# bjo5029/causal-vae

Measured on AMD Instinct MI355X. Metric: training samples/sec on 128^3 vessel volumes (3D CausalVAE train step), higher is better.
Workload: dtype bf16; 1 GPU; 3D vessel CausalVAE train step, 128^3 bf16 volumes (z-scored N(0,1)), batch 4/GPU, Adam lr 0.0001, ELBO = MSE-sum + 2000*MSE-sum(m) + KLD; global_batch=4, per_gpu_batch=4, parallelism=dp1, params=15346957

## Files before the change

causal_vae_amd/csrc/bottleneck.hip:

```cpp
#include "common.h"

#define BN_MAXM 16

namespace {

CVAE_TUNABLE(BN_NT, 0);
CVAE_TUNABLE(BN_FWD_UNROLL, 2);
CVAE_TUNABLE(BN_BWD_UNROLL, 8);
CVAE_TUNABLE(BN_FWD_SLICE, 4096);
CVAE_TUNABLE(BN_BWD_ROWS, 16);

struct TailDims { int M, N1, N2, Z, T, HM, DM, KS, P, NZ; };
struct TailParams {
    const float *b1, *W2, *b2, *Wmu, *bmu, *Wlv, *blv, *Wm0, *bm0, *gamma, *beta, *Wm3, *bm3, *Wm5, *bm5;
};
struct TailGrads {
    float *db1, *dW2, *db2, *dWmu, *dbmu, *dWlv, *dblv, *dWm0, *dbm0, *dgamma, *dbeta, *dWm3, *dbm3, *dWm5, *dbm5;
};
struct TailSaved { float *h1, *h2, *mu, *logvar, *xhat, *invstd, *a1n, *a2, *m_hat, *zm; };
struct MechFwdArgs { const float* t_onehot; float *running_mean, *running_var; long long* num_batches_tracked; float momentum, bn_eps; int bn_training;
                     const float* sync_stats; int sync_ranks; };
struct MechBwdArgs { const float *dzm_part, *g_mhat, *t_onehot; float *sync_dy, *sync_local; };
struct __attribute__((packed, aligned(4))) F4U { float x, y, z, w; };
typedef float v4f_u __attribute__((ext_vector_type(4), aligned(4)));
typedef float v2f_u __attribute__((ext_vector_type(2), aligned(4)));
struct F2U;
template <typename V> __device__ __forceinline__ V ld_stream(const float* p) {
    if constexpr (BN_NT & 1) {
        if constexpr (sizeof(V) == 16) { const v4f_u v = __builtin_nontemporal_load((const v4f_u*)p); V r; __builtin_memcpy(&r, &v, 16); return r; }
        else { const v2f_u v = __builtin_nontemporal_load((const v2f_u*)p); V r; __builtin_memcpy(&r, &v, 8); return r; }
    } else return *(const V*)p;
}
template <typename V> __device__ __forceinline__ void st_stream(float* p, const V& val) {
    if constexpr (BN_NT & 2) {
        if constexpr (sizeof(V) == 16) { v4f_u v; __builtin_memcpy(&v, &val, 16); __builtin_nontemporal_store(v, (v4f_u*)p); }
        else { v2f_u v; __builtin_memcpy(&v, &val, 8); __builtin_nontemporal_store(v, (v2f_u*)p); }
    } else *(V*)p = val;
}

template <int U>
__device__ __forceinline__ void copy_g2l(float* __restrict__ dst, const float* __restrict__ src, int n) {
    for (int base = threadIdx.x; base < n; base += 256 * U) {
        float v[U];
#pragma unroll
        for (int u = 0; u < U; ++u) v[u] = src[min(base + 256 * u, n - 1)];
#pragma unroll
        for (int u = 0; u < U; ++u) if (base + 256 * u < n) dst[base + 256 * u] = v[u];
    }
}
__device__ __forceinline__ void copy_rows_g2l(float* __restrict__ ws, const float* __restrict__ wsrc, int n, int K4, int KP) {
    constexpr int U = 8;
    for (int base = threadIdx.x * 4; base < n; base += 1024 * U) {
        float4 v[U];
#pragma unroll
        for (int u = 0; u < U; ++u) v[u] = *(const float4*)(wsrc + min(base + 1024 * u, n - 4));
#pragma unroll
        for (int u = 0; u < U; ++u) {
            const int i = base + 1024 * u;
            if (i < n) {
                const int r = i / K4, k = i - r * K4;
                float* d = ws + r * KP + k;
                d[0] = v[u].x; d[1] = v[u].y; d[2] = v[u].z; d[3] = v[u].w;
            }
        }
    }
}

struct NoiseDraw { float* eps; int n; uint64_t seed, subseq; int* counter; };
template <typename T>
__global__ __launch_bounds__(256) void pool_cat_fwd_kernel(const T* __restrict__ y, const float* __restrict__ m, float* __restrict__ t,
                                                           const long long* __restrict__ t_labels, float* __restrict__ xcat, int D, int H, int W, int C,
                                                           int OD, int OH, int OW, int m_dim, int t_dim, int K1, NoiseDraw nz) {
    const int S = OD * OH * OW, b = blockIdx.y, s = blockIdx.x;
    float* row = xcat + (size_t)b * K1;
    if (s == S) {
        if (nz.counter && b == 0) {
            const uint64_t offset = ((uint64_t)(unsigned)(*nz.counter)) << 24;
            __syncthreads();
            if (threadIdx.x == 0) *nz.counter += 1;
            for (int i = threadIdx.x; i < (nz.n + 3) / 4; i += 256) {
                float v[4];
                philox_normal4(offset + (uint64_t)i, nz.subseq, nz.seed, v);
                for (int j = 0; j < 4; ++j) if (i * 4 + j < nz.n) nz.eps[i * 4 + j] = v[j];
            }
        }
        if (t_labels) {
            const long long lab = t_labels[b];
            for (int i = threadIdx.x; i < t_dim; i += 256) { const float v = (i == lab) ? 1.f : 0.f; t[b * t_dim + i] = v; row[C * S + m_dim + i] = v; }
            for (int i = threadIdx.x; i < m_dim; i += 256) row[C * S + i] = m[b * m_dim + i];
            return;
        }
        for (int i = threadIdx.x; i < m_dim + t_dim; i += 256) row[C * S + i] = i < m_dim ? m[b * m_dim + i] : t[b * t_dim + i - m_dim];
        return;
    }
    const int ow = s % OW, oh = (s / OW) % OH, od = s / (OW * OH);
    const int d0 = pool_lo(od, D, OD), d1 = pool_hi(od, D, OD), h0 = pool_lo(oh, H, OH), h1 = pool_hi(oh, H, OH), w0 = pool_lo(ow, W, OW), w1 = pool_hi(ow, W, OW);
    const float inv = 1.f / (float)((d1 - d0) * (h1 - h0) * (w1 - w0));
    const int nh = h1 - h0, nw = w1 - w0, nvox = (d1 - d0) * nh * nw;
    for (int c = threadIdx.x; c < C; c += 256) {
        float acc = 0.f;
        constexpr int U = 8;
        for (int v0 = 0; v0 < nvox; v0 += U) {
            float v[U];
#pragma unroll
            for (int u = 0; u < U; ++u) {
                const int vi = min(v0 + u, nvox - 1), w = vi % nw, h = (vi / nw) % nh, d = vi / (nw * nh);
                v[u] = to_f32(y[((((size_t)b * D + d0 + d) * H + h0 + h) * W + w0 + w) * C + c]);
            }
#pragma unroll
            for (int u = 0; u < U; ++u) if (v0 + u < nvox) acc += v[u];
        }
        row[c * S + s] = acc * inv;
    }
}

__device__ void mech_fwd(const TailDims& d, const TailParams& p, const TailSaved& sv, const float* __restrict__ t_onehot, float* __restrict__ running_mean,
                         float* __restrict__ running_var, long long* __restrict__ num_batches_tracked, float momentum, float bn_eps, int bn_training, float* lds,
                         const float* __restrict__ sync_stats, int sync_ranks);
__device__ void mech_bwd(const TailDims& d, const TailParams& p, const TailGrads& gr, const TailSaved& sv, const float* __restrict__ dzm_part,
                         const float* __restrict__ g_mhat, const float* __restrict__ t_onehot, float* lds, float* __restrict__ sync_dy, float* __restrict__ sync_local);

template <int MT>
__global__ __launch_bounds__(256) void skinny_fwd_partial_kernel(const float* __restrict__ x, const float* __restrict__ Wt, float* __restrict__ partial,
                                                                 int M, int K, int N, int kslice, int KS, TailDims d, TailParams tp, TailSaved sv, MechFwdArgs ma) {
    extern __shared__ float dyn_lds[];
    if ((int)blockIdx.y == KS) {
        if (blockIdx.x == 0) mech_fwd(d, tp, sv, ma.t_onehot, ma.running_mean, ma.running_var, ma.num_batches_tracked, ma.momentum, ma.bn_eps, ma.bn_training, dyn_lds, ma.sync_stats, ma.sync_ranks);
        return;
    }
    constexpr int R = 4;
    const int n0 = blockIdx.x * R, ks = blockIdx.y;
    const int k0 = ks * kslice, k1 = min(K, k0 + kslice);
    float acc[R][MT];
#pragma unroll
    for (int r = 0; r < R; ++r)
#pragma unroll
        for (int mm = 0; mm < MT; ++mm) acc[r][mm] = 0.f;
    const float* wr[R];
#pragma unroll
    for (int r = 0; r < R; ++r) wr[r] = Wt + (size_t)min(n0 + r, N - 1) * K;
    const int kvec = k0 + ((k1 - k0) & ~3);
#pragma unroll BN_FWD_UNROLL
    for (int k = k0 + 4 * threadIdx.x; k < kvec; k += 1024) {
        F4U xv[MT], wv[R];
#pragma unroll
        for (int mm = 0; mm < MT; ++mm) xv[mm] = mm < M ? *(const F4U*)(x + (size_t)mm * K + k) : F4U{0.f, 0.f, 0.f, 0.f};
#pragma unroll
        for (int r = 0; r < R; ++r) wv[r] = ld_stream<F4U>(wr[r] + k);
#pragma unroll
        for (int r = 0; r < R; ++r)
#pragma unroll
            for (int mm = 0; mm < MT; ++mm) acc[r][mm] += wv[r].x * xv[mm].x + wv[r].y * xv[mm].y + wv[r].z * xv[mm].z + wv[r].w * xv[mm].w;
    }
    for (int k = kvec + threadIdx.x; k < k1; k += 256) {
#pragma unroll
        for (int r = 0; r < R; ++r)
#pragma unroll
            for (int mm = 0; mm < MT; ++mm)
                if (mm < M) acc[r][mm] += wr[r][k] * x[(size_t)mm * K + k];
    }
    __shared__ float red[4][R * MT];
    const int lane = threadIdx.x & 63, wave = threadIdx.x >> 6;
#pragma unroll
    for (int r = 0; r < R; ++r)
#pragma unroll
        for (int mm = 0; mm < MT; ++mm) {
            const float sum = wave_sum(acc[r][mm]);
            if (lane == 0) red[wave][r * MT + mm] = sum;
        }
    __syncthreads();
    if (threadIdx.x < R * MT) {
        const int r = threadIdx.x / MT, mm = threadIdx.x % MT;
        if (mm < M && n0 + r < N)
            partial[((size_t)ks * M + mm) * N + n0 + r] = red[0][threadIdx.x] + red[1][threadIdx.x] + red[2][threadIdx.x] + red[3][threadIdx.x];
    }
}


__device__ void wg_linear_fwd(const float* __restrict__ Wt, const float* __restrict__ bias, const float* xs, float* ys, float* __restrict__ yg,
                              int M, int K, int N, int act) {
    const int lane = threadIdx.x & 63, wave = threadIdx.x >> 6, nw = blockDim.x >> 6;
    for (int n = wave; n < N; n += nw) {
        float acc[BN_MAXM];
#pragma unroll
        for (int m = 0; m < BN_MAXM; ++m) acc[m] = 0.f;
        for (int k = lane; k < K; k += 64) {
            const float w = Wt[(size_t)n * K + k];
#pragma unroll
            for (int m = 0; m < BN_MAXM; ++m)
                if (m < M) acc[m] += w * xs[m * K + k];
        }
#pragma unroll
        for (int m = 0; m < BN_MAXM; ++m) {
            if (m >= M) break;
            const float s = wave_sum(acc[m]);
            if (lane == 0) {
                const float v = apply_act(s + (bias ? bias[n] : 0.f), act);
                ys[m * N + n] = v;
                if (yg) yg[(size_t)m * N + n] = v;
            }
        }
    }
}

__device__ inline float bn_bwd_dx(float k, float nb, float dy, float dbet, float xh, float dgam) { return k * fmaf(-xh, dgam, fmaf(nb, dy, -dbet)); }

__device__ void wg_linear_bwd(const float* __restrict__ Wt, float* __restrict__ dW, float* __restrict__ db, const float* gs, const float* xs, float* dxs,
                              int M, int K, int N) {
    const int T = blockDim.x;
    for (int i = threadIdx.x; i < N * K; i += T) {
        const int n = i / K, k = i - n * K;
        float acc = 0.f;
        for (int m = 0; m < M; ++m) acc += gs[m * N + n] * xs[m * K + k];
        dW[i] = acc;
    }
    if (db)
        for (int n = threadIdx.x; n < N; n += T) {
            float acc = 0.f;
            for (int m = 0; m < M; ++m) acc += gs[m * N + n];
            db[n] = acc;
        }
    if (dxs)
        for (int i = threadIdx.x; i < M * K; i += T) {
            const int m = i / K, k = i - m * K;
            float acc = 0.f;
#pragma unroll 8
            for (int n = 0; n < N; ++n) acc += gs[m * N + n] * Wt[(size_t)n * K + k];
// ... 145 lines not shown
    float* h2s = lds;
    constexpr int HO = 4;
    const int j = blockIdx.x * 4 + wave;
    float wmp[HO], wlp[HO];
#pragma unroll
    for (int u = 0; u < HO; ++u) {
        const size_t o = (size_t)min(j, d.Z - 1) * d.N2 + min(lane + 64 * u, d.N2 - 1);
        wmp[u] = p.Wmu[o]; wlp[u] = p.Wlv[o];
    }
    copy_g2l<4>(h2s, sv.h2, M * d.N2);
    __syncthreads();
    if (j >= d.Z) return;
    float am[BN_MAXM], al[BN_MAXM];
#pragma unroll
    for (int m = 0; m < BN_MAXM; ++m) { am[m] = 0.f; al[m] = 0.f; }
#pragma unroll
    for (int u = 0; u < HO; ++u) {
        const int k = lane + 64 * u;
        if (k < d.N2) {
#pragma unroll
            for (int m = 0; m < BN_MAXM; ++m)
                if (m < M) { am[m] += wmp[u] * h2s[m * d.N2 + k]; al[m] += wlp[u] * h2s[m * d.N2 + k]; }
        }
    }
    for (int k = lane + 64 * HO; k < d.N2; k += 64) {
        const float wm = p.Wmu[(size_t)j * d.N2 + k], wl = p.Wlv[(size_t)j * d.N2 + k];
#pragma unroll
        for (int m = 0; m < BN_MAXM; ++m)
            if (m < M) { am[m] += wm * h2s[m * d.N2 + k]; al[m] += wl * h2s[m * d.N2 + k]; }
    }
#pragma unroll
    for (int m = 0; m < BN_MAXM; ++m) {
        if (m >= M) break;
        const float smu = wave_sum(am[m]), slv = wave_sum(al[m]);
        if (lane == 0) {
            const float mu = smu + p.bmu[j], lv = slv + p.blv[j];
            sv.mu[m * d.Z + j] = mu; sv.logvar[m * d.Z + j] = lv;
            sv.zm[m * K4 + j] = mu + eps[m * d.Z + j] * __expf(0.5f * lv);
        }
    }
}

template <typename T>
__global__ __launch_bounds__(256) void dec_input_fwd_kernel(const float* __restrict__ zm, const float* __restrict__ Wd, const float* __restrict__ bd,
                                                            T* __restrict__ out, int M, int K4, int S, int C) {
    extern __shared__ float lds[];
    const int KP = K4 | 1;
    float* ws = lds;
    float* zs = ws + 64 * KP;
    float* part = zs + M * K4;
    const int tid = threadIdx.x;
    const size_t row0 = (size_t)blockIdx.x * 64;
    const float* wsrc = Wd + row0 * K4;
    if ((K4 & 3) == 0) copy_rows_g2l(ws, wsrc, 64 * K4, K4, KP);
    else {
        for (int i = tid; i < 64 * K4; i += 256) { const int r = i / K4, k = i - r * K4; ws[r * KP + k] = wsrc[i]; }
    }
    copy_g2l<2>(zs, zm, M * K4);
    __syncthreads();
    const int r = tid & 63, q = tid >> 6;
    const int kq = (K4 + 3) / 4, ka = q * kq, kb = min(K4, ka + kq);
    float acc[BN_MAXM];
#pragma unroll
    for (int m = 0; m < BN_MAXM; ++m) acc[m] = 0.f;
    for (int k = ka; k < kb; ++k) {
        const float w = ws[r * KP + k];
#pragma unroll
        for (int m = 0; m < BN_MAXM; ++m)
            if (m < M) acc[m] += w * zs[m * K4 + k];
    }
#pragma unroll
    for (int m = 0; m < BN_MAXM; ++m)
        if (m < M) part[(q * M + m) * 64 + r] = acc[m];
    __syncthreads();
    for (int i = tid; i < M * 64; i += 256) {
        const int m = i >> 6, rr = i & 63;
        const int n = (int)row0 + rr, c = n / S, sc = n - c * S;
        const float v = part[(0 * M + m) * 64 + rr] + part[(1 * M + m) * 64 + rr] + part[(2 * M + m) * 64 + rr] + part[(3 * M + m) * 64 + rr] + bd[n];
        out[((size_t)m * S + sc) * C + c] = from_f32<T>(v);
    }
}

template <typename T>
__global__ __launch_bounds__(256) void dec_input_bwd_kernel(const T* __restrict__ gcl, const float* __restrict__ zm, const float* __restrict__ Wd,
                                                            float* __restrict__ dWd, float* __restrict__ dbd, float* __restrict__ dzm_acc,
                                                            int M, int K4, int S, int C) {
    extern __shared__ float lds[];
    constexpr int R = 64;
    const int KP = K4 | 1;
    float* ws = lds;
    float* zs = ws + R * KP;
    float* gs = zs + M * K4;
    const int tid = threadIdx.x;
    const size_t row0 = (size_t)blockIdx.x * R;
    const float* wsrc = Wd + row0 * K4;
    float* wdst = dWd + row0 * K4;
    const bool v4 = (K4 & 3) == 0;
    {
        constexpr int UG = (BN_MAXM * R) / 256;
        float gv[UG];
#pragma unroll
        for (int u = 0; u < UG; ++u) {
            const int i = min(tid + 256 * u, M * R - 1);
            const int m = i / R, n = (int)row0 + (i - m * R), c = n / S, sc = n - c * S;
            gv[u] = to_f32(gcl[((size_t)m * S + sc) * C + c]);
        }
        if (v4) copy_rows_g2l(ws, wsrc, R * K4, K4, KP);
        else {
            for (int i = tid; i < R * K4; i += 256) { const int r = i / K4, k = i - r * K4; ws[r * KP + k] = wsrc[i]; }
        }
        copy_g2l<2>(zs, zm, M * K4);
#pragma unroll
        for (int u = 0; u < UG; ++u) if (tid + 256 * u < M * R) gs[tid + 256 * u] = gv[u];
    }
    __syncthreads();
    if (v4) {
        for (int i = tid * 4; i < R * K4; i += 1024) {
            const int r = i / K4, k = i - r * K4;
            float4 a = make_float4(0.f, 0.f, 0.f, 0.f);
            for (int m = 0; m < M; ++m) {
                const float gv = gs[m * R + r];
                const float* z = zs + m * K4 + k;
                a.x += gv * z[0]; a.y += gv * z[1]; a.z += gv * z[2]; a.w += gv * z[3];
            }
            *(float4*)(wdst + i) = a;
        }
    } else {
        for (int i = tid; i < R * K4; i += 256) {
            const int r = i / K4, k = i - r * K4;
            float acc = 0.f;
            for (int m = 0; m < M; ++m) acc += gs[m * R + r] * zs[m * K4 + k];
// ... 248 lines not shown
    const int k0 = blockIdx.x * 16;
    const int kl = tid & 15, q = tid >> 4, k = k0 + kl;
    constexpr int U = 8;
    float w0[U];
#pragma unroll
    for (int u = 0; u < U; ++u) w0[u] = p.W2[(size_t)min(q + 16 * u, N - 1) * K + min(k, K - 1)];
    copy_g2l<4>(dhs, dh2, M * N);
    for (int i = tid; i < M * 16; i += 256) h1c[i] = (k0 + (i & 15) < K) ? sv.h1[(i >> 4) * K + k0 + (i & 15)] : 0.f;
    __syncthreads();
    float acc[BN_MAXM];
#pragma unroll
    for (int m = 0; m < BN_MAXM; ++m) acc[m] = 0.f;
    if (k < K) {
        for (int n0 = q; n0 < N; n0 += 16 * U) {
            float wv[U];
#pragma unroll
            for (int u = 0; u < U; ++u) wv[u] = (n0 == q) ? w0[u] : p.W2[(size_t)min(n0 + 16 * u, N - 1) * K + k];
#pragma unroll
            for (int u = 0; u < U; ++u) {
                const int n = n0 + 16 * u;
                if (n < N) {
                    float dw = 0.f;
#pragma unroll
                    for (int m = 0; m < BN_MAXM; ++m)
                        if (m < M) { acc[m] += dhs[m * N + n] * wv[u]; dw += dhs[m * N + n] * h1c[m * 16 + kl]; }
                    gr.dW2[(size_t)n * K + k] = dw;
                }
            }
        }
    }
#pragma unroll
    for (int m = 0; m < BN_MAXM; ++m)
        if (m < M) red[(q * M + m) * 16 + kl] = acc[m];
    __syncthreads();
    if (tid < 16 && k0 + tid < K) {
        float bsum = 0.f;
        for (int m = 0; m < M; ++m) {
            float v = 0.f;
            for (int qq = 0; qq < 16; ++qq) v += red[(qq * M + m) * 16 + tid];
            v = h1c[m * 16 + tid] > 0.f ? v : 0.f;
            g1[m * K + k0 + tid] = v;
            bsum += v;
        }
        gr.db1[k0 + tid] = bsum;
    }
    if (blockIdx.x == 0)
        for (int n = tid; n < N; n += 256) {
            float b = 0.f;
            for (int m = 0; m < M; ++m) b += dhs[m * N + n];
            gr.db2[n] = b;
        }
}

struct __attribute__((packed, aligned(4))) F2U { float x, y; };
template <int MT> struct SkinnyBwdCols { static constexpr int value = 4; using vec = F4U; };
template <> struct SkinnyBwdCols<16> { static constexpr int value = 2; using vec = F2U; };
template <int MT>
__global__ __launch_bounds__(256) void skinny_bwd_colwise_kernel(const float* __restrict__ g, const float* __restrict__ x, const float* __restrict__ Wt,
                                                                 float* __restrict__ dW, float* __restrict__ dxp, int M, int K, int N, int nslice, int F, int S,
                                                                 int NS, TailDims d, TailParams tp, TailGrads tg, TailSaved sv, MechBwdArgs mb) {
    extern __shared__ float dyn_lds[];
    if ((int)blockIdx.y == NS) {
        if (blockIdx.x == 0) mech_bwd(d, tp, tg, sv, mb.dzm_part, mb.g_mhat, mb.t_onehot, dyn_lds, mb.sync_dy, mb.sync_local);
        return;
    }
    __shared__ float gs[MT][64];
    constexpr int CPT = SkinnyBwdCols<MT>::value;
    const int k0 = (blockIdx.x * 256 + threadIdx.x) * CPT, ns = blockIdx.y;
    const int n0 = ns * nslice, n1 = min(N, n0 + nslice);
    const int nk = min(CPT, K - k0);
    float xv[MT][CPT], acc[MT][CPT];
#pragma unroll
    for (int m = 0; m < MT; ++m)
#pragma unroll
        for (int c = 0; c < CPT; ++c) { xv[m][c] = (m < M && c < nk) ? x[(size_t)m * K + k0 + c] : 0.f; acc[m][c] = 0.f; }
    for (int nb = n0; nb < n1; nb += 64) {
        const int cnt = min(64, n1 - nb);
        __syncthreads();
        for (int i = threadIdx.x; i < MT * 64; i += 256) {
            const int m = i >> 6, j = i & 63;
            gs[m][j] = (m < M && j < cnt) ? g[(size_t)m * N + nb + j] : 0.f;
        }
        __syncthreads();
        if (nk == CPT) {
            constexpr int UNR = MT >= 16 ? 2 : BN_BWD_UNROLL;
#pragma unroll UNR
            for (int j = 0; j < cnt; ++j) {
                typename SkinnyBwdCols<MT>::vec w = ld_stream<typename SkinnyBwdCols<MT>::vec>(Wt + (size_t)(nb + j) * K + k0), dw;
                const float* wf = (const float*)&w;
                float* dwf = (float*)&dw;
#pragma unroll
                for (int c = 0; c < CPT; ++c) dwf[c] = 0.f;
#pragma unroll
                for (int m = 0; m < MT; ++m) {
                    const float gv = gs[m][j];
#pragma unroll
                    for (int c = 0; c < CPT; ++c) { dwf[c] += gv * xv[m][c]; acc[m][c] += gv * wf[c]; }
                }
                st_stream<typename SkinnyBwdCols<MT>::vec>(dW + (size_t)(nb + j) * K + k0, dw);
            }
        } else if (nk > 0) {
            for (int j = 0; j < cnt; ++j)
                for (int c = 0; c < nk; ++c) {
                    const float w = Wt[(size_t)(nb + j) * K + k0 + c];
                    float dw = 0.f;
#pragma unroll
                    for (int m = 0; m < MT; ++m) { dw += gs[m][j] * xv[m][c]; acc[m][c] += gs[m][j] * w; }
                    dW[(size_t)(nb + j) * K + k0 + c] = dw;
                }
        }
    }
#pragma unroll
    for (int c = 0; c < CPT; ++c) {
        const int k = k0 + c;
        if (k < F) {
            const int ch = k / S, sp = k - ch * S, C = F / S;
#pragma unroll
            for (int m = 0; m < MT; ++m)
                if (m < M) dxp[(((size_t)ns * M + m) * S + sp) * C + ch] = acc[m][c];
        }
    }
}

template <typename T>
__global__ __launch_bounds__(256) void pool_bwd_kernel(const float* __restrict__ dxp, const T* __restrict__ y, T* __restrict__ dy, int NS, int M,
                                                       int D, int H, int W, int C, int OD, int OH, int OW, int relu_mask) {
    const int S = OD * OH * OW, b = blockIdx.y, s = blockIdx.x;
    const int ow = s % OW, oh = (s / OW) % OH, od = s / (OW * OH);
    const int d0 = pool_lo(od, D, OD), d1 = pool_hi(od, D, OD), h0 = pool_lo(oh, H, OH), h1 = pool_hi(oh, H, OH), w0 = pool_lo(ow, W, OW), w1 = pool_hi(ow, W, OW);
    const int nh = h1 - h0, nw = w1 - w0, nvox = (d1 - d0) * nh * nw;
    const float inv = 1.f / (float)nvox;
    __shared__ float4 part[4][64];
    __shared__ __attribute__((aligned(16))) float val[256];
    constexpr int EPP = 16 / sizeof(T);
    const int l = threadIdx.x & 63, q = threadIdx.x >> 6;
    for (int c0 = 0; c0 < C; c0 += 256) {
        const int cw = min(256, C - c0);
        float4 a = make_float4(0.f, 0.f, 0.f, 0.f);
        if (4 * l < cw) {
            constexpr int U = 8;
            for (int n0 = q; n0 < NS; n0 += 4 * U) {
                float4 v[U];
#pragma unroll
                for (int u = 0; u < U; ++u) v[u] = *(const float4*)(dxp + (((size_t)min(n0 + 4 * u, NS - 1) * M + b) * S + s) * C + c0 + 4 * l);
#pragma unroll
                for (int u = 0; u < U; ++u)
                    if (n0 + 4 * u < NS) { a.x += v[u].x; a.y += v[u].y; a.z += v[u].z; a.w += v[u].w; }
            }
        }
        part[q][l] = a;
        __syncthreads();
        if (q == 0) {
            const float4 b1 = part[1][l], b2 = part[2][l], b3 = part[3][l];
            *(float4*)(val + 4 * l) = make_float4((a.x + b1.x + b2.x + b3.x) * inv, (a.y + b1.y + b2.y + b3.y) * inv, (a.z + b1.z + b2.z + b3.z) * inv,
                                                  (a.w + b1.w + b2.w + b3.w) * inv);
        }
        __syncthreads();
        const int ppv = cw / EPP;
        for (int i = threadIdx.x; i < nvox * ppv; i += 256) {
            const int v = i / ppv, pc = (i - v * ppv) * EPP;
            const int ww = w0 + v % nw, hh = h0 + (v / nw) % nh, dd = d0 + v / (nw * nh);
            const size_t idx = ((((size_t)b * D + dd) * H + hh) * W + ww) * C + c0 + pc;
            union { uint4 u; T e[EPP]; } mk, o;
            if (relu_mask) mk.u = *(const uint4*)(y + idx);
#pragma unroll
            for (int e = 0; e < EPP; ++e) o.e[e] = from_f32<T>((!relu_mask || to_f32(mk.e[e]) > 0.f) ? val[pc + e] : 0.f);
            *(uint4*)(dy + idx) = o.u;
        }
        __syncthreads();
    }
}

size_t mech_fwd_lds(const TailDims& d) { return sizeof(float) * (size_t)d.M * (d.T + 2 * d.HM); }
size_t mech_bwd_lds(const TailDims& d) { return sizeof(float) * ((size_t)d.M * (d.Z + d.DM + d.DM + 5 * d.HM + d.T) + 4 * 256 + 4); }
size_t fc2_fwd_lds(const TailDims& d) { return sizeof(float) * (size_t)d.M * d.N1; }
size_t mulv_fwd_lds(const TailDims& d) { return sizeof(float) * (size_t)d.M * d.N2; }
size_t mulv_bwd_lds(const TailDims& d) { return sizeof(float) * ((size_t)d.M * (d.Z + d.DM) + 2 * (size_t)d.M * d.Z + 17 * (size_t)d.M * 16 + 4 * 256 + 4); }
size_t fc2_bwd_lds(const TailDims& d) { return sizeof(float) * ((size_t)d.M * d.N2 + 17 * (size_t)d.M * 16); }
size_t bn_finish_lds(const TailDims& d) { return sizeof(float) * (size_t)d.M * (d.HM + d.T); }
size_t dec_input_fwd_lds(int M, int K4) { return sizeof(float) * ((size_t)64 * (K4 | 1) + (size_t)M * K4 + (size_t)4 * M * 64); }
size_t dec_input_bwd_lds(int M, int K4) { return sizeof(float) * ((size_t)64 * (K4 | 1) + (size_t)M * K4 + (size_t)M * 64); }
int mt_of(int M) { return M <= 4 ? 4 : (M <= 8 ? 8 : 16); }

constexpr size_t BN_LDS_MAX = 160 * 1024, BN_LDS_DEFAULT = 64 * 1024;
template <typename KERN> int bn_allow_lds(KERN kern, size_t dyn, size_t static_bytes, bool* done) {
    if (dyn <= BN_LDS_DEFAULT || *done) return CVAE_OK;
    if (hipFuncSetAttribute((const void*)kern, hipFuncAttributeMaxDynamicSharedMemorySize, (int)(BN_LDS_MAX - static_bytes)) != hipSuccess) return CVAE_E_LAUNCH;
    *done = true;
    return CVAE_OK;
}
bool lds_fwd_partial[3], lds_bwd_colwise[3], lds_fc2_fwd, lds_mulv_fwd, lds_fc2_bwd, lds_bn_finish;
constexpr size_t fwd_partial_static(int MT) { return sizeof(float) * 4 * 4 * MT; }
constexpr size_t bwd_colwise_static(int MT) { return sizeof(float) * 64 * MT; }
int fwd_lds_ready(const TailDims& d) {
    int rc;
    switch (mt_of(d.M)) {
        case 4: rc = bn_allow_lds(skinny_fwd_partial_kernel<4>, mech_fwd_lds(d), fwd_partial_static(4), &lds_fwd_partial[0]); break;
        case 8: rc = bn_allow_lds(skinny_fwd_partial_kernel<8>, mech_fwd_lds(d), fwd_partial_static(8), &lds_fwd_partial[1]); break;
        default: rc = bn_allow_lds(skinny_fwd_partial_kernel<16>, mech_fwd_lds(d), fwd_partial_static(16), &lds_fwd_partial[2]); break;
    }
    if (rc == CVAE_OK) rc = bn_allow_lds(fc2_fwd_kernel, fc2_fwd_lds(d), 0, &lds_fc2_fwd);
    if (rc == CVAE_OK) rc = bn_allow_lds(mulv_fwd_kernel, mulv_fwd_lds(d), 0, &lds_mulv_fwd);
    return rc;
}
int bwd_lds_ready(const TailDims& d) {
    int rc;
    switch (mt_of(d.M)) {
        case 4: rc = bn_allow_lds(skinny_bwd_colwise_kernel<4>, mech_bwd_lds(d), bwd_colwise_static(4), &lds_bwd_colwise[0]); break;
        case 8: rc = bn_allow_lds(skinny_bwd_colwise_kernel<8>, mech_bwd_lds(d), bwd_colwise_static(8), &lds_bwd_colwise[1]); break;
        default: rc = bn_allow_lds(skinny_bwd_colwise_kernel<16>, mech_bwd_lds(d), bwd_colwise_static(16), &lds_bwd_colwise[2]); break;
    }
    if (rc == CVAE_OK) rc = bn_allow_lds(fc2_bwd_kernel, fc2_bwd_lds(d), 0, &lds_fc2_bwd);
    return rc;
}

}

static TailDims tail_dims(const cvae_bottleneck_dims* q, int KS, int P);
static bool dims_ok(const cvae_bottleneck_dims* q) {
    if (!q) return false;
    if (q->M < 1 || q->M > BN_MAXM) return false;
    if (q->C < 64 || q->C % 64 || q->D < 1 || q->H < 1 || q->W < 1 || q->OD < 1 || q->OH < 1 || q->OW < 1) return false;
    if (q->D % q->OD || q->H % q->OH || q->W % q->OW) return false;
    if (q->m_dim < 1 || q->t_dim < 1 || q->N1 < 4 || q->N2 < 1 || q->Z < 1 || q->HM < 1 || q->HM > 1024) return false;
    if (q->Z + q->m_dim > 128 || q->N1 > 4096 || q->N2 > 2048 || q->t_dim > 65536) return false;
    const TailDims d = tail_dims(q, 0, 0);
    const int MT = mt_of(d.M), K4 = d.Z + d.DM;
    const size_t need[] = {mech_fwd_lds(d) + fwd_partial_static(MT), fc2_fwd_lds(d), mulv_fwd_lds(d), dec_input_fwd_lds(d.M, K4), dec_input_bwd_lds(d.M, K4),
                           mulv_bwd_lds(d), fc2_bwd_lds(d), mech_bwd_lds(d) + bwd_colwise_static(MT), bn_finish_lds(d)};
    for (size_t b : need)
        if (b > BN_LDS_MAX) return false;
    return true;
}
static TailDims tail_dims(const cvae_bottleneck_dims* q, int KS, int P) {
    return TailDims{(int)q->M, (int)q->N1, (int)q->N2, (int)q->Z, (int)q->t_dim, (int)q->HM, (int)q->m_dim, KS, P, (int)(q->C * q->OD * q->OH * q->OW / 64)};
}
static int fwd_ksplit(int64_t K1) { int ks = (int)(K1 / BN_FWD_SLICE); return ks < 1 ? 1 : (ks > 8 ? 8 : ks); }
static int bwd_nsplit(int64_t N1) { int ns = (int)(N1 / BN_BWD_ROWS); return ns < 1 ? 1 : (ns > 64 ? 64 : ns); }

extern "C" int cvae_bottleneck_sizes(const cvae_bottleneck_dims* q, int64_t* K1, int64_t* K4, int64_t* fwd_partial_floats, int64_t* dzm_partial_floats,
                                     int64_t* dx_partial_floats) {
    if (!dims_ok(q)) return CVAE_E_BADSHAPE;
    const int64_t S = q->OD * q->OH * q->OW, F = q->C * S, k1 = F + q->m_dim + q->t_dim, k4 = q->Z + q->m_dim;
    if (K1) *K1 = k1;
    if (K4) *K4 = k4;
    if (fwd_partial_floats) *fwd_partial_floats = (int64_t)fwd_ksplit(k1) * q->M * q->N1;
    if (dzm_partial_floats) *dzm_partial_floats = (F / 64) * q->M * k4;
    if (dx_partial_floats) *dx_partial_floats = (int64_t)bwd_nsplit(q->N1) * q->M * F;
    return CVAE_OK;
}

template <int MT>
static void launch_fwd_partial(const float* x, const float* W1, float* partial, int M, int K, int N, int KS, const TailDims& d, const TailParams& p, const TailSaved& sv,
                               const MechFwdArgs& ma, hipStream_t st) {
    const int kslice = (K + KS - 1) / KS;
    hipLaunchKernelGGL(skinny_fwd_partial_kernel<MT>, dim3((unsigned)((N + 3) / 4), (unsigned)(KS + 1)), dim3(256), mech_fwd_lds(d), st, x, W1, partial, M, K, N, kslice,
                       KS, d, p, sv, ma);
}
template <int MT>
static void launch_bwd_colwise(const float* g, const float* x, const float* W1, float* dW, float* dxp, int M, int K, int N, int NS, int F, int S, const TailDims& d,
                               const TailParams& p, const TailGrads& tg, const TailSaved& sv, const MechBwdArgs& mb, hipStream_t st) {
    const int nslice = (N + NS - 1) / NS;
    hipLaunchKernelGGL(skinny_bwd_colwise_kernel<MT>, dim3((unsigned)((K + 256 * SkinnyBwdCols<MT>::value - 1) / (256 * SkinnyBwdCols<MT>::value)), (unsigned)(NS + 1)), dim3(256), mech_bwd_lds(d), st, g, x, W1, dW, dxp, M, K, N,
                       nslice, F, S, NS, d, p, tg, sv, mb);
}

extern "C" int cvae_bottleneck_bn_local_stats(const float* Wm0, const float* bm0, const float* t_onehot, const int64_t* t_labels, float* local_stats, int64_t M, int64_t t_dim,
                                              int64_t HM, void* stream) {
    if (M < 1 || M > BN_MAXM || t_dim < 1 || HM < 1 || HM > 1024) return CVAE_E_BADSHAPE;
    if (!Wm0 || !bm0 || !local_stats || (!t_onehot && !t_labels)) return CVAE_E_NULLPTR;
    hipLaunchKernelGGL(mech_bn_local_stats_kernel, dim3(1), dim3(256), 0, (hipStream_t)stream, Wm0, bm0, t_onehot, (const long long*)t_labels, local_stats, (int)M, (int)t_dim, (int)HM);
    CVAE_CHECK_LAUNCH();
    return CVAE_OK;
}

extern "C" int cvae_bottleneck_fwd(const cvae_bottleneck_dims* q, const cvae_bottleneck_params* w, const void* y_cl, const float* m, float* t_onehot,
                                   const int64_t* t_labels, float* eps, float* running_mean, float* running_var, long long* num_batches_tracked, float momentum,
                                   float bn_eps, int bn_training, float* xcat, float* partial, float* dzm_acc, const cvae_bottleneck_saved* sv, void* dec_cl, int dtype,
                                   const float* bn_rank_stats, int bn_ranks, const cvae_bottleneck_noise* noise, void* stream) {
    if (!dims_ok(q)) return CVAE_E_BADSHAPE;
    if (noise && !noise->call_counter) return CVAE_E_NULLPTR;
    const NoiseDraw nz = noise ? NoiseDraw{eps, (int)(q->M * q->Z), noise->seed, noise->subsequence, noise->call_counter} : NoiseDraw{nullptr, 0, 0, 0, nullptr};
    if (bn_rank_stats && (bn_ranks < 1 || !bn_training)) return CVAE_E_BADSHAPE;
    if (dtype != CVAE_F32 && dtype != CVAE_BF16) return CVAE_E_DTYPE;
    if (!w || !sv || !y_cl || !m || !t_onehot || !eps || !xcat || !partial || !dec_cl) return CVAE_E_NULLPTR;
    if (bn_training && q->M * (bn_rank_stats ? bn_ranks : 1) < 2) return CVAE_E_BADSHAPE;
    if (!bn_training && (!running_mean || !running_var)) return CVAE_E_NULLPTR;
    if (fwd_lds_ready(tail_dims(q, 0, 0)) != CVAE_OK) return CVAE_E_LAUNCH;
    hipStream_t st = (hipStream_t)stream;
    const int M = (int)q->M, S = (int)(q->OD * q->OH * q->OW), C = (int)q->C, F = C * S;
    const int K1 = F + (int)q->m_dim + (int)q->t_dim, K4 = (int)(q->Z + q->m_dim), KS = fwd_ksplit(K1);
    if (dtype == CVAE_BF16)
        hipLaunchKernelGGL(pool_cat_fwd_kernel<bf16>, dim3(S + 1, M), dim3(256), 0, st, (const bf16*)y_cl, m, t_onehot, (const long long*)t_labels, xcat, (int)q->D, (int)q->H, (int)q->W, C,
                           (int)q->OD, (int)q->OH, (int)q->OW, (int)q->m_dim, (int)q->t_dim, K1, nz);
    else
        hipLaunchKernelGGL(pool_cat_fwd_kernel<float>, dim3(S + 1, M), dim3(256), 0, st, (const float*)y_cl, m, t_onehot, (const long long*)t_labels, xcat, (int)q->D, (int)q->H, (int)q->W, C,
                           (int)q->OD, (int)q->OH, (int)q->OW, (int)q->m_dim, (int)q->t_dim, K1, nz);
    CVAE_CHECK_LAUNCH();
    const TailDims d = tail_dims(q, KS, 0);
    const TailParams p{w->b1, w->W2, w->b2, w->Wmu, w->bmu, w->Wlv, w->blv, w->Wm0, w->bm0, w->gamma, w->beta, w->Wm3, w->bm3, w->Wm5, w->bm5};
    const TailSaved s{sv->h1, sv->h2, sv->mu, sv->logvar, sv->xhat, sv->invstd, sv->a1n, sv->a2, sv->m_hat, sv->zm};
    const MechFwdArgs ma{t_onehot, running_mean, running_var, num_batches_tracked, momentum, bn_eps, bn_training, bn_rank_stats, bn_ranks};
    if (M <= 4) launch_fwd_partial<4>(xcat, w->W1, partial, M, K1, (int)q->N1, KS, d, p, s, ma, st);
    else if (M <= 8) launch_fwd_partial<8>(xcat, w->W1, partial, M, K1, (int)q->N1, KS, d, p, s, ma, st);
    else launch_fwd_partial<16>(xcat, w->W1, partial, M, K1, (int)q->N1, KS, d, p, s, ma, st);
    CVAE_CHECK_LAUNCH();
    hipLaunchKernelGGL(fc2_fwd_kernel, dim3((unsigned)((q->N2 + 3) / 4)), dim3(256), fc2_fwd_lds(d), st, d, p, s, (const float*)partial);
    CVAE_CHECK_LAUNCH();
    hipLaunchKernelGGL(mulv_fwd_kernel, dim3((unsigned)((q->Z + 3) / 4)), dim3(256), mulv_fwd_lds(d), st, d, p, s, eps);
    CVAE_CHECK_LAUNCH();
    const size_t lds_d = dec_input_fwd_lds(M, K4);
    if (dtype == CVAE_BF16)
        hipLaunchKernelGGL(dec_input_fwd_kernel<bf16>, dim3(C * S / 64), dim3(256), lds_d, st, (const float*)sv->zm, w->Wd, w->bd, (bf16*)dec_cl, M, K4, S, C);
    else
        hipLaunchKernelGGL(dec_input_fwd_kernel<float>, dim3(C * S / 64), dim3(256), lds_d, st, (const float*)sv->zm, w->Wd, w->bd, (float*)dec_cl, M, K4, S, C);
    CVAE_CHECK_LAUNCH();
    return CVAE_OK;
// ... 63 lines not shown
```

Baseline: 5213 samples/s.

## Restructure skinny bottleneck GEMV kernels with aligned vector loads and interleaved row groups

The forward skinny kernel now gives each block R rows interleaved by a stride of 4, splits K into 256-wide aligned chunks after peeling to 16-byte alignment, and batches CH chunks of loads ahead of compute using a sched_barrier. The backward colwise kernel drops its LDS staging of g and broadcasts g values through readlane. It also walks interleaved row groups with unrolled vector weight loads and handles unaligned peel and tail columns. The split factors change as well, aiming at more memory-level parallelism and aligned wide loads on the large fc1 weight, at the cost of more complex index handling and register pressure.

```diff
diff --git a/causal_vae_amd/csrc/bottleneck.hip b/causal_vae_amd/csrc/bottleneck.hip
--- a/causal_vae_amd/csrc/bottleneck.hip
+++ b/causal_vae_amd/csrc/bottleneck.hip
@@ -5,10 +5,6 @@
 namespace {
 
 CVAE_TUNABLE(BN_NT, 0);
-CVAE_TUNABLE(BN_FWD_UNROLL, 2);
-CVAE_TUNABLE(BN_BWD_UNROLL, 8);
-CVAE_TUNABLE(BN_FWD_SLICE, 4096);
-CVAE_TUNABLE(BN_BWD_ROWS, 16);
 
 struct TailDims { int M, N1, N2, Z, T, HM, DM, KS, P, NZ; };
 struct TailParams {
@@ -22,19 +18,20 @@
                      const float* sync_stats; int sync_ranks; };
 struct MechBwdArgs { const float *dzm_part, *g_mhat, *t_onehot; float *sync_dy, *sync_local; };
 struct __attribute__((packed, aligned(4))) F4U { float x, y, z, w; };
-typedef float v4f_u __attribute__((ext_vector_type(4), aligned(4)));
-typedef float v2f_u __attribute__((ext_vector_type(2), aligned(4)));
-struct F2U;
+template <int N> struct ExtVec { typedef float type __attribute__((ext_vector_type(N))); };
+template <> struct ExtVec<1> { typedef float type; };
 template <typename V> __device__ __forceinline__ V ld_stream(const float* p) {
     if constexpr (BN_NT & 1) {
-        if constexpr (sizeof(V) == 16) { const v4f_u v = __builtin_nontemporal_load((const v4f_u*)p); V r; __builtin_memcpy(&r, &v, 16); return r; }
-        else { const v2f_u v = __builtin_nontemporal_load((const v2f_u*)p); V r; __builtin_memcpy(&r, &v, 8); return r; }
+        using E = typename ExtVec<sizeof(V) / 4>::type;
+        const E v = __builtin_nontemporal_load((const E*)p);
+        V r; __builtin_memcpy(&r, &v, sizeof(V)); return r;
     } else return *(const V*)p;
 }
 template <typename V> __device__ __forceinline__ void st_stream(float* p, const V& val) {
     if constexpr (BN_NT & 2) {
-        if constexpr (sizeof(V) == 16) { v4f_u v; __builtin_memcpy(&v, &val, 16); __builtin_nontemporal_store(v, (v4f_u*)p); }
-        else { v2f_u v; __builtin_memcpy(&v, &val, 8); __builtin_nontemporal_store(v, (v2f_u*)p); }
+        using E = typename ExtVec<sizeof(V) / 4>::type;
+        E v; __builtin_memcpy(&v, &val, sizeof(V));
+        __builtin_nontemporal_store(v, (E*)p);
     } else *(V*)p = val;
 }
 
@@ -120,47 +117,78 @@
 __device__ void mech_bwd(const TailDims& d, const TailParams& p, const TailGrads& gr, const TailSaved& sv, const float* __restrict__ dzm_part,
                          const float* __restrict__ g_mhat, const float* __restrict__ t_onehot, float* lds, float* __restrict__ sync_dy, float* __restrict__ sync_local);
 
+template <int MT> struct SkinnyFwdCfg { static constexpr int R = 8, CH = 3; };
+template <> struct SkinnyFwdCfg<8> { static constexpr int R = 8, CH = 1; };
+template <> struct SkinnyFwdCfg<16> { static constexpr int R = 4, CH = 1; };
+template <int CPT> __device__ __forceinline__ int peel_of(const float* p) { return (int)((CPT - (((uintptr_t)p >> 2) & (CPT - 1))) & (CPT - 1)); }
+
 template <int MT>
 __global__ __launch_bounds__(256) void skinny_fwd_partial_kernel(const float* __restrict__ x, const float* __restrict__ Wt, float* __restrict__ partial,
-                                                                 int M, int K, int N, int kslice, int KS, TailDims d, TailParams tp, TailSaved sv, MechFwdArgs ma) {
+                                                                 int M, int K, int N, int KS, TailDims d, TailParams tp, TailSaved sv, MechFwdArgs ma) {
     extern __shared__ float dyn_lds[];
     if ((int)blockIdx.y == KS) {
         if (blockIdx.x == 0) mech_fwd(d, tp, sv, ma.t_onehot, ma.running_mean, ma.running_var, ma.num_batches_tracked, ma.momentum, ma.bn_eps, ma.bn_training, dyn_lds, ma.sync_stats, ma.sync_ranks);
         return;
     }
-    constexpr int R = 4;
-    const int n0 = blockIdx.x * R, ks = blockIdx.y;
-    const int k0 = ks * kslice, k1 = min(K, k0 + kslice);
+    constexpr int R = SkinnyFwdCfg<MT>::R, CH = SkinnyFwdCfg<MT>::CH;
+    const int tid = threadIdx.x, ks = blockIdx.y;
+    const int n0 = 4 * R * (int)(blockIdx.x >> 2) + (int)(blockIdx.x & 3);
+    if (n0 >= N) return;
+    const float* wr[R];
+#pragma unroll
+    for (int r = 0; r < R; ++r) wr[r] = Wt + (size_t)(n0 + 4 * r < N ? n0 + 4 * r : n0) * K;
+    const int peel = min(peel_of<4>(wr[0]), K), nvec = (K - peel) >> 2, nch = (nvec + 255) >> 8;
+    const int c0 = (int)((long long)nch * ks / KS), c1 = (int)((long long)nch * (ks + 1) / KS);
+    int ke = -1;
+    if (ks == 0 && tid < 8) {
+        ke = tid < 4 ? tid : peel + 4 * nvec + tid - 4;
+        if (tid < 4 ? tid >= peel : ke >= K) ke = -1;
+    }
     float acc[R][MT];
 #pragma unroll
     for (int r = 0; r < R; ++r)
 #pragma unroll
         for (int mm = 0; mm < MT; ++mm) acc[r][mm] = 0.f;
-    const float* wr[R];
-#pragma unroll
-    for (int r = 0; r < R; ++r) wr[r] = Wt + (size_t)min(n0 + r, N - 1) * K;
-    const int kvec = k0 + ((k1 - k0) & ~3);
-#pragma unroll BN_FWD_UNROLL
-    for (int k = k0 + 4 * threadIdx.x; k < kvec; k += 1024) {
-        F4U xv[MT], wv[R];
-#pragma unroll
-        for (int mm = 0; mm < MT; ++mm) xv[mm] = mm < M ? *(const F4U*)(x + (size_t)mm * K + k) : F4U{0.f, 0.f, 0.f, 0.f};
-#pragma unroll
-        for (int r = 0; r < R; ++r) wv[r] = ld_stream<F4U>(wr[r] + k);
+    for (int cb = c0; cb < c1; cb += CH) {
+        float4 wv[CH][R];
+        F4U xv[CH][MT];
+        bool live[CH];
+#pragma unroll
+        for (int u = 0; u < CH; ++u) {
+            const int j = (cb + u) * 256 + tid;
+            live[u] = cb + u < c1 && j < nvec;
+            const int k = peel + 4 * min(j, nvec - 1);
+#pragma unroll
+            for (int r = 0; r < R; ++r) wv[u][r] = ld_stream<float4>(wr[r] + k);
+#pragma unroll
+            for (int mm = 0; mm < MT; ++mm) xv[u][mm] = *(const F4U*)(x + (size_t)min(mm, M - 1) * K + k);
+        }
+        __builtin_amdgcn_sched_barrier(0);
+#pragma unroll
+        for (int u = 0; u < CH; ++u)
+#pragma unroll
+            for (int mm = 0; mm < MT; ++mm)
+                if (!(live[u] && mm < M)) xv[u][mm] = F4U{0.f, 0.f, 0.f, 0.f};
+#pragma unroll
+        for (int u = 0; u < CH; ++u)
+#pragma unroll
+            for (int r = 0; r < R; ++r)
+#pragma unroll
+                for (int mm = 0; mm < MT; ++mm) acc[r][mm] += wv[u][r].x * xv[u][mm].x + wv[u][r].y * xv[u][mm].y + wv[u][r].z * xv[u][mm].z + wv[u][r].w * xv[u][mm].w;
+    }
+    if (ke >= 0) {
+        float we[R], xe[MT];
+#pragma unroll
+        for (int r = 0; r < R; ++r) we[r] = wr[r][ke];
+#pragma unroll
+        for (int mm = 0; mm < MT; ++mm) xe[mm] = mm < M ? x[(size_t)mm * K + ke] : 0.f;
 #pragma unroll
         for (int r = 0; r < R; ++r)
 #pragma unroll
-            for (int mm = 0; mm < MT; ++mm) acc[r][mm] += wv[r].x * xv[mm].x + wv[r].y * xv[mm].y + wv[r].z * xv[mm].z + wv[r].w * xv[mm].w;
-    }
-    for (int k = kvec + threadIdx.x; k < k1; k += 256) {
-#pragma unroll
-        for (int r = 0; r < R; ++r)
-#pragma unroll
-            for (int mm = 0; mm < MT; ++mm)
-                if (mm < M) acc[r][mm] += wr[r][k] * x[(size_t)mm * K + k];
+            for (int mm = 0; mm < MT; ++mm) acc[r][mm] += we[r] * xe[mm];
     }
     __shared__ float red[4][R * MT];
-    const int lane = threadIdx.x & 63, wave = threadIdx.x >> 6;
+    const int lane = tid & 63, wave = tid >> 6;
 #pragma unroll
     for (int r = 0; r < R; ++r)
 #pragma unroll
@@ -169,10 +197,10 @@
             if (lane == 0) red[wave][r * MT + mm] = sum;
         }
     __syncthreads();
-    if (threadIdx.x < R * MT) {
-        const int r = threadIdx.x / MT, mm = threadIdx.x % MT;
-        if (mm < M && n0 + r < N)
-            partial[((size_t)ks * M + mm) * N + n0 + r] = red[0][threadIdx.x] + red[1][threadIdx.x] + red[2][threadIdx.x] + red[3][threadIdx.x];
+    if (tid < R * MT) {
+        const int r = tid / MT, mm = tid % MT;
+        if (mm < M && n0 + 4 * r < N)
+            partial[((size_t)ks * M + mm) * N + n0 + 4 * r] = red[0][tid] + red[1][tid] + red[2][tid] + red[3][tid];
     }
 }
 
@@ -424,6 +452,7 @@
     const int tid = threadIdx.x;
     const size_t row0 = (size_t)blockIdx.x * 64;
     const float* wsrc = Wd + row0 * K4;
+    const float bias = bd[row0 + (tid & 63)];
     if ((K4 & 3) == 0) copy_rows_g2l(ws, wsrc, 64 * K4, K4, KP);
     else {
         for (int i = tid; i < 64 * K4; i += 256) { const int r = i / K4, k = i - r * K4; ws[r * KP + k] = wsrc[i]; }
@@ -448,7 +477,7 @@
     for (int i = tid; i < M * 64; i += 256) {
         const int m = i >> 6, rr = i & 63;
         const int n = (int)row0 + rr, c = n / S, sc = n - c * S;
-        const float v = part[(0 * M + m) * 64 + rr] + part[(1 * M + m) * 64 + rr] + part[(2 * M + m) * 64 + rr] + part[(3 * M + m) * 64 + rr] + bd[n];
+        const float v = part[(0 * M + m) * 64 + rr] + part[(1 * M + m) * 64 + rr] + part[(2 * M + m) * 64 + rr] + part[(3 * M + m) * 64 + rr] + bias;
         out[((size_t)m * S + sc) * C + c] = from_f32<T>(v);
     }
 }
@@ -803,68 +832,72 @@
         }
 }
 
-struct __attribute__((packed, aligned(4))) F2U { float x, y; };
-template <int MT> struct SkinnyBwdCols { static constexpr int value = 4; using vec = F4U; };
-template <> struct SkinnyBwdCols<16> { static constexpr int value = 2; using vec = F2U; };
+template <int MT> struct SkinnyBwdCfg { static constexpr int CPT = 4, UR = 64 / MT; };
+template <> struct SkinnyBwdCfg<16> { static constexpr int CPT = 2, UR = 4; };
+template <int NC> struct VecOf { using type = float; };
+template <> struct VecOf<2> { using type = float2; };
+template <> struct VecOf<4> { using type = float4; };
+
 template <int MT>
 __global__ __launch_bounds__(256) void skinny_bwd_colwise_kernel(const float* __restrict__ g, const float* __restrict__ x, const float* __restrict__ Wt,
-                                                                 float* __restrict__ dW, float* __restrict__ dxp, int M, int K, int N, int nslice, int F, int S,
+                                                                 float* __restrict__ dW, float* __restrict__ dxp, int M, int K, int N, int RW, int F, int S,
                                                                  int NS, TailDims d, TailParams tp, TailGrads tg, TailSaved sv, MechBwdArgs mb) {
     extern __shared__ float dyn_lds[];
     if ((int)blockIdx.y == NS) {
         if (blockIdx.x == 0) mech_bwd(d, tp, tg, sv, mb.dzm_part, mb.g_mhat, mb.t_onehot, dyn_lds, mb.sync_dy, mb.sync_local);
         return;
     }
-    __shared__ float gs[MT][64];
-    constexpr int CPT = SkinnyBwdCols<MT>::value;
-    const int k0 = (blockIdx.x * 256 + threadIdx.x) * CPT, ns = blockIdx.y;
-    const int n0 = ns * nslice, n1 = min(N, n0 + nslice);
-    const int nk = min(CPT, K - k0);
+    constexpr int CPT = SkinnyBwdCfg<MT>::CPT, UR = SkinnyBwdCfg<MT>::UR;
+    using V = typename VecOf<CPT>::type;
+    const int ns = blockIdx.y, ph = ns & 3, n0 = 4 * RW * (ns >> 2) + ph;
+    const int peel = min(peel_of<CPT>(Wt + (size_t)ph * K), K), nvec = (K - peel) / CPT;
+    const int j = blockIdx.x * 256 + threadIdx.x;
+    const bool full = j < nvec;
+    const int k0 = full ? peel + CPT * j : (j - nvec < peel ? j - nvec : CPT * nvec + (j - nvec));
+    const int nc = full ? CPT : (k0 < K ? 1 : 0);
     float xv[MT][CPT], acc[MT][CPT];
 #pragma unroll
     for (int m = 0; m < MT; ++m)
 #pragma unroll
-        for (int c = 0; c < CPT; ++c) { xv[m][c] = (m < M && c < nk) ? x[(size_t)m * K + k0 + c] : 0.f; acc[m][c] = 0.f; }
-    for (int nb = n0; nb < n1; nb += 64) {
-        const int cnt = min(64, n1 - nb);
-        __syncthreads();
-        for (int i = threadIdx.x; i < MT * 64; i += 256) {
-            const int m = i >> 6, j = i & 63;
-            gs[m][j] = (m < M && j < cnt) ? g[(size_t)m * N + nb + j] : 0.f;
-        }
-        __syncthreads();
-        if (nk == CPT) {
-            constexpr int UNR = MT >= 16 ? 2 : BN_BWD_UNROLL;
-#pragma unroll UNR
-            for (int j = 0; j < cnt; ++j) {
-                typename SkinnyBwdCols<MT>::vec w = ld_stream<typename SkinnyBwdCols<MT>::vec>(Wt + (size_t)(nb + j) * K + k0), dw;
-                const float* wf = (const float*)&w;
-                float* dwf = (float*)&dw;
-#pragma unroll
-                for (int c = 0; c < CPT; ++c) dwf[c] = 0.f;
-#pragma unroll
-                for (int m = 0; m < MT; ++m) {
-                    const float gv = gs[m][j];
-#pragma unroll
-                    for (int c = 0; c < CPT; ++c) { dwf[c] += gv * xv[m][c]; acc[m][c] += gv * wf[c]; }
-                }
-                st_stream<typename SkinnyBwdCols<MT>::vec>(dW + (size_t)(nb + j) * K + k0, dw);
-            }
-        } else if (nk > 0) {
-            for (int j = 0; j < cnt; ++j)
-                for (int c = 0; c < nk; ++c) {
-                    const float w = Wt[(size_t)(nb + j) * K + k0 + c];
-                    float dw = 0.f;
-#pragma unroll
-                    for (int m = 0; m < MT; ++m) { dw += gs[m][j] * xv[m][c]; acc[m][c] += gs[m][j] * w; }
-                    dW[(size_t)(nb + j) * K + k0 + c] = dw;
-                }
+        for (int c = 0; c < CPT; ++c) { xv[m][c] = (m < M && c < nc) ? x[(size_t)m * K + k0 + c] : 0.f; acc[m][c] = 0.f; }
+    const int lane = threadIdx.x & 63, gu = lane / MT, gm = lane % MT;
+    for (int i0 = 0; i0 < RW; i0 += UR) {
+        const int gn = n0 + 4 * (i0 + gu);
+        const float gl = (i0 + gu < RW && gn < N && gm < M) ? g[(size_t)gm * N + gn] : 0.f;
+        float w[UR][CPT];
+#pragma unroll
+        for (int u = 0; u < UR; ++u) {
+            const int n = n0 + 4 * (i0 + u);
+            const float* wp = Wt + (size_t)((i0 + u < RW && n < N) ? n : ph) * K + k0;
+#pragma unroll
+            for (int c = 0; c < CPT; ++c) w[u][c] = 0.f;
+            if (full) { const V v = ld_stream<V>(wp); __builtin_memcpy(w[u], &v, sizeof(V)); }
+            else if (nc) w[u][0] = *wp;
+        }
+        __builtin_amdgcn_sched_barrier(0);
+#pragma unroll
+        for (int u = 0; u < UR; ++u) {
+            const int n = n0 + 4 * (i0 + u);
+            float dw[CPT];
+#pragma unroll
+            for (int c = 0; c < CPT; ++c) dw[c] = 0.f;
+#pragma unroll
+            for (int m = 0; m < MT; ++m) {
+                const float gv = __builtin_bit_cast(float, __builtin_amdgcn_readlane(__builtin_bit_cast(int, gl), u * MT + m));
+#pragma unroll
+                for (int c = 0; c < CPT; ++c) { dw[c] += gv * xv[m][c]; acc[m][c] += gv * w[u][c]; }
+            }
+            if (i0 + u < RW && n < N) {
+                float* dp = dW + (size_t)n * K + k0;
+                if (full) { V v; __builtin_memcpy(&v, dw, sizeof(V)); st_stream<V>(dp, v); }
+                else if (nc) *dp = dw[0];
+            }
         }
     }
 #pragma unroll
     for (int c = 0; c < CPT; ++c) {
         const int k = k0 + c;
-        if (k < F) {
+        if (c < nc && k < F) {
             const int ch = k / S, sp = k - ch * S, C = F / S;
 #pragma unroll
             for (int m = 0; m < MT; ++m)
@@ -941,8 +974,8 @@
     return CVAE_OK;
 }
 bool lds_fwd_partial[3], lds_bwd_colwise[3], lds_fc2_fwd, lds_mulv_fwd, lds_fc2_bwd, lds_bn_finish;
-constexpr size_t fwd_partial_static(int MT) { return sizeof(float) * 4 * 4 * MT; }
-constexpr size_t bwd_colwise_static(int MT) { return sizeof(float) * 64 * MT; }
+constexpr size_t fwd_partial_static(int MT) { return sizeof(float) * 4 * (MT == 4 ? SkinnyFwdCfg<4>::R * 4 : MT == 8 ? SkinnyFwdCfg<8>::R * 8 : SkinnyFwdCfg<16>::R * 16); }
+constexpr size_t bwd_colwise_static(int) { return 0; }
 int fwd_lds_ready(const TailDims& d) {
     int rc;
     switch (mt_of(d.M)) {
@@ -986,8 +1019,9 @@
 static TailDims tail_dims(const cvae_bottleneck_dims* q, int KS, int P) {
     return TailDims{(int)q->M, (int)q->N1, (int)q->N2, (int)q->Z, (int)q->t_dim, (int)q->HM, (int)q->m_dim, KS, P, (int)(q->C * q->OD * q->OH * q->OW / 64)};
 }
-static int fwd_ksplit(int64_t K1) { int ks = (int)(K1 / BN_FWD_SLICE); return ks < 1 ? 1 : (ks > 8 ? 8 : ks); }
-static int bwd_nsplit(int64_t N1) { int ns = (int)(N1 / BN_BWD_ROWS); return ns < 1 ? 1 : (ns > 64 ? 64 : ns); }
+static int fwd_ksplit(int64_t K1) { int ks = (int)(K1 / 2048); return ks < 1 ? 1 : (ks > 8 ? 8 : ks); }
+static int bwd_groups(int64_t N1) { int g = (int)((N1 + 63) / 64); return g < 1 ? 1 : (g > 16 ? 16 : g); }
+static int bwd_nsplit(int64_t N1) { return 4 * bwd_groups(N1); }
 
 extern "C" int cvae_bottleneck_sizes(const cvae_bottleneck_dims* q, int64_t* K1, int64_t* K4, int64_t* fwd_partial_floats, int64_t* dzm_partial_floats,
                                      int64_t* dx_partial_floats) {
@@ -1004,16 +1038,17 @@
 template <int MT>
 static void launch_fwd_partial(const float* x, const float* W1, float* partial, int M, int K, int N, int KS, const TailDims& d, const TailParams& p, const TailSaved& sv,
                                const MechFwdArgs& ma, hipStream_t st) {
-    const int kslice = (K + KS - 1) / KS;
-    hipLaunchKernelGGL(skinny_fwd_partial_kernel<MT>, dim3((unsigned)((N + 3) / 4), (unsigned)(KS + 1)), dim3(256), mech_fwd_lds(d), st, x, W1, partial, M, K, N, kslice,
-                       KS, d, p, sv, ma);
+    constexpr int R = SkinnyFwdCfg<MT>::R;
+    hipLaunchKernelGGL(skinny_fwd_partial_kernel<MT>, dim3((unsigned)(4 * ((N + 4 * R - 1) / (4 * R))), (unsigned)(KS + 1)), dim3(256), mech_fwd_lds(d), st, x, W1, partial, M, K,
+                       N, KS, d, p, sv, ma);
 }
 template <int MT>
 static void launch_bwd_colwise(const float* g, const float* x, const float* W1, float* dW, float* dxp, int M, int K, int N, int NS, int F, int S, const TailDims& d,
                                const TailParams& p, const TailGrads& tg, const TailSaved& sv, const MechBwdArgs& mb, hipStream_t st) {
-    const int nslice = (N + NS - 1) / NS;
-    hipLaunchKernelGGL(skinny_bwd_colwise_kernel<MT>, dim3((unsigned)((K + 256 * SkinnyBwdCols<MT>::value - 1) / (256 * SkinnyBwdCols<MT>::value)), (unsigned)(NS + 1)), dim3(256), mech_bwd_lds(d), st, g, x, W1, dW, dxp, M, K, N,
-                       nslice, F, S, NS, d, p, tg, sv, mb);
+    constexpr int CPT = SkinnyBwdCfg<MT>::CPT;
+    const int G = NS / 4, RW = ((N + 3) / 4 + G - 1) / G;
+    hipLaunchKernelGGL(skinny_bwd_colwise_kernel<MT>, dim3((unsigned)((K / CPT + 2 * (CPT - 1) + 255) / 256), (unsigned)(NS + 1)), dim3(256), mech_bwd_lds(d), st, g, x, W1, dW,
+                       dxp, M, K, N, RW, F, S, NS, d, p, tg, sv, mb);
 }
 
 extern "C" int cvae_bottleneck_bn_local_stats(const float* Wm0, const float* bm0, const float* t_onehot, const int64_t* t_labels, float* local_stats, int64_t M, int64_t t_dim,
```

Result: slower. 5152 samples/s (-1.2%).
